# bruniss/multi-task-3d-resencoder-unet

Measured on AMD Instinct MI355X. Metric: train patches/sec (b,c,z,y,x) ResEncM 1x128^3, higher is better.
Workload: dtype bf16; 1 GPU; cfg2: ResEncM (6 stages, feats [32, 64, 128, 256, 512, 512], blocks [1, 3, 4, 6, 6, 6]), 1-in, heads ['sheet'], patch 128x128x128, batch 2/GPU, full train step (fwd+loss+bwd+allreduce+clip+AdamW); global_batch=2, parallelism=dp1

## Files before the change

### include/rxunet.h

```cpp
#ifndef RXUNET_H
#define RXUNET_H

#include <stddef.h>
#include <stdint.h>

#ifdef __cplusplus
extern "C" {
#endif

#define RX_OK 0
#define RX_EINVAL (-1)
#define RX_EUNSUPPORTED (-2)
#define RX_ELAUNCH (-3)
#define RX_EWORKSPACE (-4)

typedef enum { RX_F32 = 0, RX_BF16 = 1, RX_F16 = 2 } rx_dtype;
typedef enum { RX_ACT_NONE = 0, RX_ACT_SIGMOID = 1, RX_ACT_SOFTMAX = 2 } rx_head_act;

typedef struct {
  void* ptr;
  int32_t n, z, y, x, c, ld;
  int64_t cs;
} rx_act;

// ... 10 lines not shown
                  const int* taps, void* const* w_fwd, void* const* w_bwd, void* stream);

size_t rx_conv_workspace_hint(void);
int rx_conv3d_fwd(rx_dtype dt, const rx_act* x, const void* w_fwd, const float* bias, const rx_act* y,
                  const int32_t kernel[3], const int32_t stride[3], void* ws, size_t ws_bytes, void* stream);
int rx_conv3d_fwd_stats(rx_dtype dt, const rx_act* x, const void* w_fwd, const float* bias, const rx_act* y,
                        const int32_t kernel[3], const int32_t stride[3], float eps, float* stats, void* ws,
                        size_t ws_bytes, void* stream);
int rx_conv3d_bwd_data(rx_dtype dt, const rx_act* dy, const void* w_bwd, const rx_act* dx,
                       const int32_t kernel[3], const int32_t stride[3], int accumulate, void* ws,
                       size_t ws_bytes, void* stream);
int rx_conv3d_bwd_data_instats(rx_dtype dt, const rx_act* dy, const void* w_bwd, const rx_act* dx,
                               const int32_t kernel[3], const int32_t stride[3], int accumulate, const rx_act* in_y,
                               const float* in_stats, float slope, float* m12, int* fused, void* ws, size_t ws_bytes,
                               void* stream);
size_t rx_conv3d_bwd_weight_workspace(const rx_act* x, const rx_act* dy, const int32_t kernel[3]);
int rx_conv3d_bwd_weight(rx_dtype dt, const rx_act* x, const rx_act* dy, float* dw, const int32_t kernel[3],
                         const int32_t stride[3], void* ws, size_t ws_bytes, void* stream);

int rx_convT3d_fwd(rx_dtype dt, const rx_act* x, const void* w_fwd, const float* bias, const rx_act* y,
                   const int32_t stride[3], void* ws, size_t ws_bytes, void* stream);
int rx_convT3d_bwd_data(rx_dtype dt, const rx_act* dy, const void* w_bwd, const rx_act* dx,
                        const int32_t stride[3], int accumulate, void* ws, size_t ws_bytes, void* stream);
size_t rx_convT3d_bwd_weight_workspace(const rx_act* x, const rx_act* dy, const int32_t stride[3]);
int rx_convT3d_bwd_weight(rx_dtype dt, const rx_act* x, const rx_act* dy, float* dw, const int32_t stride[3],
                          void* ws, size_t ws_bytes, void* stream);

size_t rx_instnorm_stats_workspace(const rx_act* y);
int rx_instnorm_stats(rx_dtype dt, const rx_act* y, float eps, float* stats, void* ws, size_t ws_bytes,
                      void* stream);
// ... 249 lines not shown
```

### multi-task-3d-resencoder-unet_amd/csrc/build.py

```python
import os
import subprocess
import sys

HERE = os.path.dirname(os.path.abspath(__file__))
SOURCES = ["rx_runtime.hip", "rx_instnorm.hip", "rx_head.hip", "rx_stem.hip", "rx_pack_optim.hip", "rx_igemm.hip", "rx_wgrad.hip", "rx_wgrad_halo.hip", "rx_conv_halo.hip", "rx_stem_wgrad.hip", "rx_loss.hip", "rx_se.hip", "rx_dgrad_s2.hip", "rx_prog.hip", "rx_pointwise.hip", "rx_infer.hip", "rx_augment.hip", "rx_geometry.hip", "rx_morph.hip", "rx_patchsearch.hip", "rx_ingest.hip", "rx_affine.hip", "rx_metrics.hip", "rx_elastic.hip", "rx_preview.hip", "rx_meshslice.hip", "rx_surface.hip"]
HEADERS = ["rx_common.h", "rx_internal.h", "rx_reduce.h", "rx_instnorm_core.h", "rx_prog.h", "rx_affine_core.h", "rx_elastic_core.h", "rx_meshslice_core.h", "rx_conv_halo_plan.h", os.path.join("..", "..", "include", "rxunet.h")]
LIB = os.path.join(HERE, "librxunet.so")
HIPCC = os.environ.get("HIPCC", "/opt/rocm/bin/hipcc")
FLAGS = ["-O3", "--offload-arch=gfx950", "-std=c++17", "-fPIC", "-Wno-unused-result"]


def _stale(target, deps):
    if not os.path.exists(target):
        return True
    t = os.path.getmtime(target)
    return any(os.path.getmtime(d) > t for d in deps)


def build(force=False, verbose=True):
    hdrs = [os.path.join(HERE, h) for h in HEADERS] + [os.path.abspath(__file__)]
    objs = []
    procs = []
    for src in SOURCES:
        obj = os.path.join(HERE, src.replace(".hip", ".o"))
# ... 20 lines not shown
```

### multi-task-3d-resencoder-unet_amd/engine/lib.py

```python
import ctypes
import os
from ctypes import POINTER, c_char_p, c_double, c_float, c_int, c_int32, c_long, c_size_t, c_void_p

import torch

_HERE = os.path.dirname(os.path.abspath(__file__))
LIB_PATH = os.environ.get("RX_LIBRARY") or os.path.join(os.path.dirname(_HERE), "csrc", "librxunet.so")

RX_F32, RX_BF16, RX_F16 = 0, 1, 2
RX_ACT_NONE, RX_ACT_SIGMOID, RX_ACT_SOFTMAX = 0, 1, 2
DTYPE_CODE = {torch.float32: RX_F32, torch.bfloat16: RX_BF16, torch.float16: RX_F16}
RX_SW_U8, RX_SW_U16, RX_SW_F32 = 0, 1, 2
RX_SW_SCALE, RX_SW_ZSCORE = 0, 1
RX_SW_BLEND_AVERAGE, RX_SW_BLEND_UNIT, RX_SW_BLEND_NONE = 0, 1, 2
RX_SW_CAST_U8, RX_SW_CAST_U16 = 0, 1
RX_AUG_PW_NONE, RX_AUG_PW_AFFINE, RX_AUG_PW_PLANE, RX_AUG_PW_NOISE = 0, 1, 2, 3
RX_AUG_G3_NONE, RX_AUG_G3_FILTER, RX_AUG_G3_DOWNSCALE = 0, 1, 2
RX_AUG_MAX_K, RX_AUG_MAX_BOXES = 21, 4
RX_LOSS_BCE_LOGITS, RX_LOSS_BCE_PROB, RX_LOSS_MSE = 0, 1, 2
RX_REDUCE_MEAN, RX_REDUCE_SUM = 0, 1
RX_INGEST_COPY, RX_INGEST_DIV255, RX_INGEST_DIV65535, RX_INGEST_NORMAL_U16, RX_INGEST_NORMAL_MUL2 = 0, 1, 2, 3, 4
RX_AFFINE_LINEAR, RX_AFFINE_NEAREST = 0, 1
RX_AFFINE_CONSTANT, RX_AFFINE_CLAMP = 0, 1
RX_EDT_NONE, RX_EDT_MAX_EXTENT = 1 << 30, 1024
# ... 23 lines not shown

_SIGNATURES = {
    "rx_abi_version": (c_int, []),
    "rx_last_error": (c_char_p, []),
    "rx_device_arch_ok": (c_int, []),
    "rx_last_conv_kernel": (c_char_p, []),
    "rx_pack_conv_weight": (c_int, [c_int, c_void_p, c_int, c_int, c_int, c_void_p, c_void_p, c_void_p]),
    "rx_pack_convT_weight": (c_int, [c_int, c_void_p, c_int, c_int, c_int, c_void_p, c_void_p, c_void_p]),
    "rx_pack_multi": (c_int, [c_int, c_int, c_void_p, c_void_p, c_void_p, c_void_p, c_void_p, c_void_p, c_void_p, c_void_p]),
    "rx_conv_workspace_hint": (c_size_t, []),
    "rx_conv3d_fwd": (c_int, [c_int, _P, c_void_p, c_void_p, _P, I3, I3, c_void_p, c_size_t, c_void_p]),
    "rx_conv3d_fwd_stats": (c_int, [c_int, _P, c_void_p, c_void_p, _P, I3, I3, c_float, c_void_p, c_void_p, c_size_t, c_void_p]),
    "rx_conv3d_bwd_data": (c_int, [c_int, _P, c_void_p, _P, I3, I3, c_int, c_void_p, c_size_t, c_void_p]),
    "rx_conv3d_bwd_data_instats": (c_int, [c_int, _P, c_void_p, _P, I3, I3, c_int, _P, c_void_p, c_float, c_void_p, POINTER(c_int),
                                           c_void_p, c_size_t, c_void_p]),
    "rx_instnorm_act_bwd_apply": (c_int, [c_int, _P, _P, c_void_p, _P, c_float, c_void_p, _P, _P, c_int, c_void_p]),
    "rx_conv3d_bwd_weight_workspace": (c_size_t, [_P, _P, I3]),
    "rx_conv3d_bwd_weight": (c_int, [c_int, _P, _P, c_void_p, I3, I3, c_void_p, c_size_t, c_void_p]),
    "rx_convT3d_fwd": (c_int, [c_int, _P, c_void_p, c_void_p, _P, I3, c_void_p, c_size_t, c_void_p]),
    "rx_convT3d_bwd_data": (c_int, [c_int, _P, c_void_p, _P, I3, c_int, c_void_p, c_size_t, c_void_p]),
    "rx_convT3d_bwd_weight_workspace": (c_size_t, [_P, _P, I3]),
    "rx_convT3d_bwd_weight": (c_int, [c_int, _P, _P, c_void_p, I3, c_void_p, c_size_t, c_void_p]),
    "rx_instnorm_stats_workspace": (c_size_t, [_P]),
    "rx_instnorm_stats": (c_int, [c_int, _P, c_float, c_void_p, c_void_p, c_size_t, c_void_p]),
    "rx_instnorm_act_fwd": (c_int, [c_int, _P, c_void_p, _P, _P, c_float, c_void_p]),
    "rx_instnorm_stats_mask": (c_int, [c_void_p, c_void_p, c_int, c_void_p]),
    "rx_instnorm_fwd": (c_int, [c_int, _P, c_float, c_void_p, _P, _P, c_float, c_void_p, c_size_t, c_void_p]),
    "rx_instnorm_act_bwd": (c_int, [c_int, _P, _P, c_void_p, _P, c_float, _P, _P, c_int, c_void_p, c_size_t,
                                    c_void_p]),
    "rx_instnorm_act_bwd_res": (c_int, [c_int, _P, _P, c_void_p, _P, c_float, _P, I3, _P, _P, c_void_p, c_size_t, c_void_p]),
# ... 158 lines not shown
```

### multi-task-3d-resencoder-unet_amd/engine/ops/__init__.py

```python
from ctypes import byref, c_int32, c_void_p

import numpy as np
import torch

from .. import lib as _l
from ..lib import I3, RxAct, check, load, stream_ptr
from . import core, infer, losses, mesh, network, pipeline, validation
from .core import (_U16, Act, LaunchProfiler, Program, event_free, event_new, event_record, profiling,
                   set_profiler, stream_wait, timed_bytes, workspace)
from .infer import (SW_ACT, SW_BLEND, SW_CAST, SW_NORM, sw_accumulate, sw_finalize, sw_gather,
                    sw_gather_workspace, sw_occupancy)
from .losses import (bce_dice_loss_bwd, bce_dice_loss_fwd, cross_entropy_loss_bwd, cross_entropy_loss_fwd,
                     elem_loss_bwd, elem_loss_fwd, masked_cosine_loss_bwd, masked_cosine_loss_fwd)
from .mesh import mesh_slice_labels, mesh_slice_normals
from .network import (avgpool_bwd, avgpool_fwd, channel_sum, conv3d_bwd_data, conv3d_bwd_data_instats,
                      conv3d_bwd_weight, conv3d_fwd, conv3d_fwd_stats, convT3d_bwd_data, convT3d_bwd_weight, convT3d_fwd,
                      head_bwd, head_fwd, instnorm_act_bwd, instnorm_act_bwd_apply, instnorm_act_bwd_head,
                      instnorm_act_bwd_res, instnorm_act_fwd, instnorm_act_head_fwd, instnorm_act_pool_fwd, instnorm_fwd,
                      instnorm_gate_act_bwd, instnorm_gate_act_fwd, instnorm_stats, instnorm_stats_mask, pack_conv_weight,
                      pack_convT_weight, pack_weights_multi, se_gate_bwd, se_gate_fwd, se_workspace_bytes,
                      stem_conv_bwd_weight, stem_conv_fwd, stem_conv_fwd_stats)
from .pipeline import (affine_apply, affine_table, aug_filter_zy, aug_philox_u32, aug_pointwise, augment_batch,
                       box_stats, elastic_apply, elastic_nodes, elastic_tables, geom_apply, geom_table, ingest, label_dilate)
from .validation import (class_counts, edt_sq, mask_edges, normal_stats, preview_frames, preview_panel, seg_counts,
                         surface_hist, surface_scratch)
```

### multi-task-3d-resencoder-unet_amd/engine/ops/network.py

```python
import ctypes
from ctypes import byref, c_int

import torch

from .. import lib as _l
from ..lib import I3, check, load, stream_ptr
from .core import LaunchProfiler, _code, _desc, _ptr, _tb, _ws_args, flops, hbm, timed_bytes, workspace


def _pack_bytes(w, dtype, want_fwd, want_bwd):
    e = torch.empty((), dtype=dtype).element_size()
    return w.numel() * (4 + (e if want_fwd else 0) + (e if want_bwd else 0))


def _pack(entry, w, co, ci, dtype, w_fwd, w_bwd, want_fwd, want_bwd):
    taps = w[0, 0].numel()
    if want_fwd and w_fwd is None:
        w_fwd = torch.empty((taps, co, ci), dtype=dtype, device=w.device)
    if want_bwd and w_bwd is None:
        w_bwd = torch.empty((taps, ci, co), dtype=dtype, device=w.device)
    check(getattr(load(), entry)(_code(dtype), _ptr(w), w.shape[0], w.shape[1], taps, _ptr(w_fwd if want_fwd else None),
                                 _ptr(w_bwd if want_bwd else None), stream_ptr()), entry)
    return w_fwd, w_bwd

# ... 49 lines not shown
@flops(lambda dy, dx, kernel: _igemm("dgrad", dx, dy, dx, kernel))
def conv3d_bwd_data(dy, w_bwd, dx, kernel, stride, accumulate=False, ws=None):
    check(load().rx_conv3d_bwd_data(_code(dy.dtype), byref(dy.desc()), _ptr(w_bwd), byref(dx.desc()), I3(*kernel), I3(*stride),
                                    int(accumulate), *_ws_args(ws), stream_ptr()), "rx_conv3d_bwd_data")


@flops(lambda dy, dx, kernel: _igemm("dgrad", dx, dx, dy, kernel))
def conv3d_bwd_data_instats(dy, w_bwd, dx, kernel, stride, accumulate, in_y, in_stats, slope, m12, ws=None):
    fused = c_int(0)
    check(load().rx_conv3d_bwd_data_instats(_code(dy.dtype), byref(dy.desc()), _ptr(w_bwd), byref(dx.desc()), I3(*kernel),
                                            I3(*stride), int(accumulate), byref(in_y.desc()), _ptr(in_stats), float(slope),
                                            _ptr(m12), byref(fused), *_ws_args(ws), stream_ptr()), "rx_conv3d_bwd_data_instats")
    return bool(fused.value)


def _bwd_bytes(g, y, out, dy, d_residual, accumulate_residual):
    return _tb(g) + _tb(y) + _tb(dy) + _tb(out) + _tb(d_residual) * (2 if accumulate_residual else 1)


@hbm("in_act_bwd_apply", _bwd_bytes)
def instnorm_act_bwd_apply(g, y, stats, out, dy, m12, slope=0.01, d_residual=None, accumulate_residual=False):
    check(load().rx_instnorm_act_bwd_apply(_code(y.dtype), byref(g.desc()), byref(y.desc()), _ptr(stats), _desc(out), float(slope),
                                           _ptr(m12), byref(dy.desc()), _desc(d_residual), int(accumulate_residual), stream_ptr()),
          "rx_instnorm_act_bwd_apply")


@flops(lambda x, dy, kernel: (f"wgrad:wgrad_kernel<{64 if dy.c % 64 == 0 else 32},{64 if x.c % 64 == 0 else 32}>",
                              _conv_flops(dy, x, kernel)))
def conv3d_bwd_weight(x, dy, dw, kernel, stride, ws=None):
    need = load().rx_conv3d_bwd_weight_workspace(byref(x.desc()), byref(dy.desc()), I3(*kernel))
# ... 177 lines not shown
```

### multi-task-3d-resencoder-unet_amd/engine/plan.py

```python
import contextlib
import os
from dataclasses import dataclass
from typing import Callable, ClassVar, Dict, List, NamedTuple, Optional

import torch
from torch import nn

from . import lib as _l
from . import ops
from .ops import Act


class UnsupportedConfig(NotImplementedError):
    pass


_SIDE_STREAMS: Dict[str, "torch.cuda.Stream"] = {}


def side_stream(device):
    key = str(device)
    st = _SIDE_STREAMS.get(key)
    if st is None:
        st = _SIDE_STREAMS[key] = torch.cuda.Stream(device=device)
# ... 82 lines not shown


@dataclass(eq=False)
class ConvRec:
    kind: ClassVar[str] = "conv"
    x: AT
    y: AT
    pk: dict
    b: Optional[torch.Tensor]
    widx: int
    bidx: Optional[int]
    kernel: list
    stride: list
    stats_to: Optional["InactRec"] = None
    instats_for: Optional["InactRec"] = None


@dataclass(eq=False)
class ConvTRec:
    kind: ClassVar[str] = "convT"
    x: AT
    y: AT
    pk: dict
    b: Optional[torch.Tensor]
    widx: int
    bidx: Optional[int]
    stride: list
    cat: AT


@dataclass(eq=False)
class InactRec:
    kind: ClassVar[str] = "inact"
    y: AT
    stats: torch.Tensor
    eps: float
    res: Optional[AT]
    out: AT
    slope: float
    gate: Optional[Gate]
    drop: Optional[Drop]
    stats_done: bool = False
    pool_to: Optional["PoolRec"] = None
    head_to: Optional["HeadRec"] = None
    head_src: Optional["HeadRec"] = None
    head_dw_fused: bool = False
    m12: Optional[torch.Tensor] = None
    m12_valid: bool = False
    m12x: Optional[torch.Tensor] = None


@dataclass(eq=False)
class PoolRec:
    kind: ClassVar[str] = "pool"
    x: AT
    y: AT
    stride: list
# ... 489 lines not shown
                                [((slice(None), slice(0, head.in_channels)), (slice(None), slice(None)))])
            tape.append(HeadRec(x=low, w=hw_k, b=head.bias, widx=self._param(head.weight), bidx=self._param(head.bias), k=k,
                                name=name, out=out, act=act_code))

        self._gen_forward()
        if self.needs_grad:
            self._gen_backward()

    def _fuse_conv_stats(self, tape):
        for rec, nxt in zip(tape, tape[1:]):
            if (rec.kind == "conv" and nxt.kind == "inact" and nxt.y is rec.y and self.dtype != torch.float32
                    and list(rec.kernel) == [3, 3, 3] and list(rec.stride) == [1, 1, 1]
                    and _above_single_launch(rec.y.act) and _halo_x_ok(rec.y.act)):
                rec.stats_to, nxt.stats_done = nxt, True

    def _fuse_stem_stats(self, tape):
        for rec, nxt in zip(tape, tape[1:]):
            if (rec.kind == "stem" and nxt.kind == "inact" and nxt.y is rec.y and self.dtype != torch.float32
                    and _above_single_launch(rec.y.act)):
                rec.stats_to, nxt.stats_done = nxt, True

    def _fuse_block_pool(self, tape):
        producers = {id(r.out): r for r in tape if r.kind == "inact" and r.gate is None}
        for rec in tape:
            if rec.kind == "pool" and id(rec.x) in producers and _above_single_launch(rec.x.act):
                src = producers[id(rec.x)]
                if src.pool_to is None:
                    src.pool_to, rec.fused = rec, True

    def _fuse_head(self, tape):
# ... 15 lines not shown
        def step():
            st = r.stats_to
            if st is not None:
                ops.stem_conv_fwd_stats(self._x, r.w, r.b, r.y.act, r.kernel, st.stats, self._eps_now(st))
                self._mask_dropped(st)
            else:
                ops.stem_conv_fwd(self._x, r.w, r.b, r.y.act, r.kernel)
        return [step]

    def _fwd_image(self, r: ImageRec):
        return [lambda: ops.stem_conv_fwd(self._x, r.w, None, r.y.act, [1, 1, 1])]

    def _fwd_conv(self, r: ConvRec):
        def step():
            self._await_pack(r.pk)
            st = r.stats_to
            if st is not None:
                ops.conv3d_fwd_stats(r.x.act, r.pk["w_fwd"], r.b, r.y.act, r.kernel, r.stride, st.stats, self._eps_now(st))
                self._mask_dropped(st)
            else:
                ops.conv3d_fwd(r.x.act, r.pk["w_fwd"], r.b, r.y.act, r.kernel, r.stride)
        return [step]

    def _fwd_convT(self, r: ConvTRec):
        def step():
            self._await_pack(r.pk)
            ops.convT3d_fwd(r.x.act, r.pk["w_fwd"], r.b, r.y.act, r.stride)
        return [step]

    def _fwd_inact(self, r: InactRec):
        res = r.res.act if r.res is not None else None
        g, head, pool = r.gate, r.head_to, r.pool_to
# ... 18 lines not shown
            ops.instnorm_act_head_fwd(r.y.act, r.stats, r.out.act if keep else None, head.w.view(head.k, -1), head.b, head.out,
                                      head.act if self._apply_act else _l.RX_ACT_NONE, r.slope)

        def with_pool():
            stats_pass()
            ops.instnorm_act_pool_fwd(r.y.act, r.stats, r.out.act, pool.y.act, pool.stride, r.slope, res)

        def plain():
            if r.stats_done:
                ops.instnorm_act_fwd(r.y.act, r.stats, r.out.act, r.slope, res)
            elif r.drop is not None and r.drop.active:
                stats_pass()
                ops.instnorm_act_fwd(r.y.act, r.stats, r.out.act, r.slope, res)
            else:
                ops.instnorm_fwd(r.y.act, r.stats, r.out.act, r.slope, res, r.eps)
        if g is not None:
            return [gated]
        return [with_head if head is not None else with_pool if pool is not None else plain]

    def _fwd_pool(self, r: PoolRec):
        return [] if r.fused else [lambda: ops.avgpool_fwd(r.x.act, r.y.act, r.stride)]

    def _fwd_copy(self, r: CopyRec):
        return [lambda: ops.avgpool_fwd(r.x.act, r.y.act, (1, 1, 1))]

    def _fwd_head(self, r: HeadRec):
        if r.fwd_fused:
            return []
        return [lambda: ops.head_fwd(r.x.act, r.w.view(r.k, -1), r.b, r.out, r.act if self._apply_act else _l.RX_ACT_NONE)]

# ... 1 lines not shown
        f = self.fwd
        self.n_fwd_enc = None
        self.fwd_dec_start = []
        build = {StemRec: self._fwd_stem, ImageRec: self._fwd_image, ConvRec: self._fwd_conv, ConvTRec: self._fwd_convT,
                 InactRec: self._fwd_inact, PoolRec: self._fwd_pool, CopyRec: self._fwd_copy, HeadRec: self._fwd_head}
        full_res = self.spatial[0] * self.spatial[1] * self.spatial[2]
        for tape in [self.enc_tape] + self.dec_tapes:
            if tape is not self.enc_tape:
                if self.n_fwd_enc is None:
                    self.n_fwd_enc = len(f)
                self.fwd_dec_start.append(len(f))
            self._fuse_conv_stats(tape)
            self._fuse_stem_stats(tape)
            self._fuse_block_pool(tape)
            self._fuse_head(tape)
            for rec in tape:
                if (tape is self.enc_tape and self._pack_delay_at is None and rec.kind in ("conv", "pool")
                        and rec.y.act.voxels < full_res):
                    self._pack_delay_at = len(f)
                f += build[type(rec)](rec)

    def _dy_for(self, y: AT):
        key = (y.act.dims, y.act.c)
        turn = self._dy_turn.get(key, 0)
        self._dy_turn[key] = (turn + 1) % self.dy_ring
        slot = key + (turn,)
        if slot not in self.dy_pool:
            t = torch.empty((*y.act.dims, y.act.c), dtype=self.dtype, device=self.device)
            self.bytes_alloc += t.numel() * t.element_size()
            self.dy_pool[slot] = Act(t)
# ... 105 lines not shown
        gres, acc = None, False
        if res is not None and res.needs_grad:
            gres, acc = self._claim_grad(res, r)
        plain16 = r.gate is None and res is None and self.dtype != torch.float32 and _above_single_launch(out.act)
        last = out.last_writer
        if plain16 and isinstance(last, HeadRec):
            heads = [h for h in tape if h.kind == "head" and h.x is out]
            if len(heads) == 1 and heads[0].k <= 4:
                r.head_src, last.dx_fused = heads[0], True
                if heads[0].fwd_fused and heads[0].w is self.params[heads[0].widx]:
                    r.head_dw_fused, last.dw_fused = True, True
        if (plain16 and isinstance(last, ConvRec) and out.act.full_buffer and out.act.root is None and out.act.c % 32 == 0
                and _halo_x_ok(out.act)):
            r.m12 = torch.empty((self.B, out.act.c, 2), dtype=torch.float32, device=self.device)
            last.instats_for = r
        if r.gate is not None:
            return [self._bwd_inact_gated(r, gout, dy, gres, acc)]
        pend, out.pool_pending = out.pool_pending, None
        if gres is not None and not acc and _above_single_launch(y.act):
            return [self._bwd_inact_res(r, gout, dy, gres, pend)]
        steps = []
        if pend is not None:
            steps.append(lambda: ops.avgpool_bwd(pend.gy, pend.gx, pend.stride, True))
        return steps + [self._bwd_inact_plain(r, gout, dy, gres, acc)]

    def _bwd_inact_gated(self, r, gout, dy, gres, acc):
        g = r.gate

        def step():
            self._before_dy_write(dy)
# ... 51 lines not shown
        def wlaunch(dw, ws):
            if r.kind == "stem":
                ops.stem_conv_bwd_weight(self._x, dy, dw, r.kernel, ws)
            elif "wgrad" not in self._skip:
                ops.conv3d_bwd_weight(r.x.act, dy, dw, r.kernel, r.stride, ws)
        steps = [self._wgrad_step(r, dy, wlaunch)]
        if r.kind == "conv" and r.x.needs_grad:
            gx, acc = self._claim_grad(r.x, r)
            if r.x.act.full_buffer:
                self._cat_written[r.x.act.key] = True

            def dstep():
                if "dgrad" in self._skip:
                    return
                ia = r.instats_for
                if ia is None:
                    ops.conv3d_bwd_data(dy, r.pk["w_bwd"], gx, r.kernel, r.stride, acc)
                else:
                    ia.m12_valid = ops.conv3d_bwd_data_instats(dy, r.pk["w_bwd"], gx, r.kernel, r.stride, acc, ia.y.act, ia.stats,
                                                               ia.slope, ia.m12)
            steps.append(dstep)
        return steps

    def _bwd_convT(self, r: ConvTRec, tape, i):
        if not self._view_written(r.y):
            raise RuntimeError("plan bug: concat gradient not initialised before the transposed conv")
        gy = self._cat_grad(r)
        gx, acc = self._claim_grad(r.x, r)
        wstep = self._wgrad_step(r, gy, lambda dw, ws: ops.convT3d_bwd_weight(r.x.act, gy, dw, r.stride, ws))

        def step():
# ... 465 lines not shown
```

Before: 117.0 patches/s.

## Add fused small-volume conv+instnorm kernels for deep low-resolution stages

Adds a dedicated HIP kernel for 3x3x3 stride-1 convs on volumes of at most 64 voxels. One workgroup holds a whole sample's activations in LDS, splits K across waves, and fuses the instance-norm statistics plus normalize/activation/residual into the forward conv. In backward, the dgrad kernel is fused with the preceding instnorm backward and residual-gradient accumulation. The aim is to remove separate launches and round trips through memory at the tiny 4^3 bottleneck stages. The cost is a new code path whose grid parallelism is small (N*Co/16 blocks), so it could underuse the GPU.

```diff
diff --git a/include/rxunet.h b/include/rxunet.h
--- a/include/rxunet.h
+++ b/include/rxunet.h
@@ -48,6 +48,15 @@
                                const int32_t kernel[3], const int32_t stride[3], int accumulate, const rx_act* in_y,
                                const float* in_stats, float slope, float* m12, int* fused, void* ws, size_t ws_bytes,
                                void* stream);
+int rx_conv_small_select(rx_dtype dt, int z, int y, int x, int ci, int co, const int32_t kernel[3],
+                         const int32_t stride[3]);
+int rx_conv3d_in_fwd_small(rx_dtype dt, const rx_act* x, const void* w_fwd, const float* bias, const rx_act* y,
+                           const int32_t kernel[3], const int32_t stride[3], float eps, float* stats,
+                           const rx_act* residual, const rx_act* out, float slope, void* stream);
+int rx_conv3d_bwd_data_in_small(rx_dtype dt, const rx_act* dy, const void* w_bwd, const rx_act* dx,
+                                const int32_t kernel[3], const int32_t stride[3], int accumulate, const rx_act* in_y,
+                                const float* in_stats, const rx_act* in_out, float slope, const rx_act* in_dy,
+                                const rx_act* d_residual, int accumulate_residual, void* stream);
 size_t rx_conv3d_bwd_weight_workspace(const rx_act* x, const rx_act* dy, const int32_t kernel[3]);
 int rx_conv3d_bwd_weight(rx_dtype dt, const rx_act* x, const rx_act* dy, float* dw, const int32_t kernel[3],
                          const int32_t stride[3], void* ws, size_t ws_bytes, void* stream);
diff --git a/multi-task-3d-resencoder-unet_amd/csrc/build.py b/multi-task-3d-resencoder-unet_amd/csrc/build.py
--- a/multi-task-3d-resencoder-unet_amd/csrc/build.py
+++ b/multi-task-3d-resencoder-unet_amd/csrc/build.py
@@ -3,7 +3,7 @@
 import sys
 
 HERE = os.path.dirname(os.path.abspath(__file__))
-SOURCES = ["rx_runtime.hip", "rx_instnorm.hip", "rx_head.hip", "rx_stem.hip", "rx_pack_optim.hip", "rx_igemm.hip", "rx_wgrad.hip", "rx_wgrad_halo.hip", "rx_conv_halo.hip", "rx_stem_wgrad.hip", "rx_loss.hip", "rx_se.hip", "rx_dgrad_s2.hip", "rx_prog.hip", "rx_pointwise.hip", "rx_infer.hip", "rx_augment.hip", "rx_geometry.hip", "rx_morph.hip", "rx_patchsearch.hip", "rx_ingest.hip", "rx_affine.hip", "rx_metrics.hip", "rx_elastic.hip", "rx_preview.hip", "rx_meshslice.hip", "rx_surface.hip"]
+SOURCES = ["rx_runtime.hip", "rx_instnorm.hip", "rx_head.hip", "rx_stem.hip", "rx_pack_optim.hip", "rx_igemm.hip", "rx_conv_small.hip", "rx_wgrad.hip", "rx_wgrad_halo.hip", "rx_conv_halo.hip", "rx_stem_wgrad.hip", "rx_loss.hip", "rx_se.hip", "rx_dgrad_s2.hip", "rx_prog.hip", "rx_pointwise.hip", "rx_infer.hip", "rx_augment.hip", "rx_geometry.hip", "rx_morph.hip", "rx_patchsearch.hip", "rx_ingest.hip", "rx_affine.hip", "rx_metrics.hip", "rx_elastic.hip", "rx_preview.hip", "rx_meshslice.hip", "rx_surface.hip"]
 HEADERS = ["rx_common.h", "rx_internal.h", "rx_reduce.h", "rx_instnorm_core.h", "rx_prog.h", "rx_affine_core.h", "rx_elastic_core.h", "rx_meshslice_core.h", "rx_conv_halo_plan.h", os.path.join("..", "..", "include", "rxunet.h")]
 LIB = os.path.join(HERE, "librxunet.so")
 HIPCC = os.environ.get("HIPCC", "/opt/rocm/bin/hipcc")
diff --git a/multi-task-3d-resencoder-unet_amd/csrc/rx_conv_small.hip b/multi-task-3d-resencoder-unet_amd/csrc/rx_conv_small.hip
--- /dev/null
+++ b/multi-task-3d-resencoder-unet_amd/csrc/rx_conv_small.hip
@@ -0,0 +1,409 @@
+#include "rx_common.h"
+#include "rx_internal.h"
+#include "rx_reduce.h"
+#include "rx_instnorm_core.h"
+
+constexpr int CS_MAXV = 64;
+constexpr int CS_BN = 16;
+constexpr int CS_NW = 8;
+constexpr int CS_RING = 8;
+constexpr int CS_KU = 64;
+constexpr int CS_MAXCI = 1024;
+constexpr int CS_STAGE = 16 * CS_KU * 2;
+
+struct CsArgs {
+  const void* in;
+  const void* w;
+  int ldi;
+  long in_ss;
+  int Z, Y, X, V, Ci, Co, N, flip;
+  void* o;
+  int ldo;
+  long o_ss;
+  const float* bias;
+  int accumulate;
+  float* stats_w;
+  const float* stats_r;
+  float eps, slope;
+  const void* res;
+  int ldr;
+  long r_ss;
+  void* out;
+  int ldout;
+  long out_ss;
+  const void* iy;
+  int ldiy;
+  long iy_ss;
+  const void* iout;
+  int ldio;
+  long io_ss;
+  void* dy;
+  int lddy;
+  long dy_ss;
+  void* dres;
+  int lddr;
+  long dr_ss;
+  int acc_res, mask;
+};
+
+template <typename T>
+struct Mma16;
+template <>
+struct Mma16<bf16_t> {
+  __device__ static inline void run(f32x4& c, const u32x4& a, const u32x4& b) {
+    c = __builtin_amdgcn_mfma_f32_16x16x32_bf16(__builtin_bit_cast(bf16x8, a), __builtin_bit_cast(bf16x8, b), c, 0, 0, 0);
+  }
+};
+template <>
+struct Mma16<f16_t> {
+  __device__ static inline void run(f32x4& c, const u32x4& a, const u32x4& b) {
+    c = __builtin_amdgcn_mfma_f32_16x16x32_f16(__builtin_bit_cast(f16x8, a), __builtin_bit_cast(f16x8, b), c, 0, 0, 0);
+  }
+};
+
+template <typename T>
+struct alignas(8) Vec8 {
+  T v[4];
+};
+template <typename T>
+__device__ inline Vec8<T> ld8(const T* p) {
+  Vec8<T> r;
+  *reinterpret_cast<u32x2*>(&r) = *reinterpret_cast<const u32x2*>(p);
+  return r;
+}
+template <typename T>
+__device__ inline void st8(T* p, const Vec8<T>& r) {
+  *reinterpret_cast<u32x2*>(p) = *reinterpret_cast<const u32x2*>(&r);
+}
+
+static size_t cs_lds_main(int Ci) {
+  const size_t act = (size_t)(CS_MAXV + 1) * Ci * 2 + (size_t)CS_NW * CS_STAGE, part = (size_t)CS_NW * CS_MAXV * CS_BN * sizeof(float);
+  return act > part ? act : part;
+}
+static size_t cs_lds_bytes(int Ci) { return cs_lds_main(Ci) + 4 * 2 * CS_BN * sizeof(double) + 2 * CS_BN * sizeof(float); }
+
+template <typename T, bool BWD>
+__global__ __launch_bounds__(CS_NW * 64) void conv_small_kernel(const CsArgs a, int lds_main) {
+  extern __shared__ __attribute__((aligned(16))) unsigned char cs_smem[];
+  u32x4* sX = reinterpret_cast<u32x4*>(cs_smem);
+  float* part = reinterpret_cast<float*>(cs_smem);
+  double* red = reinterpret_cast<double*>(cs_smem + lds_main);
+  float* pr = reinterpret_cast<float*>(cs_smem + lds_main + 4 * 2 * CS_BN * sizeof(double));
+
+  const int tid = threadIdx.x, lane = tid & 63, wave = __builtin_amdgcn_readfirstlane(tid >> 6);
+  const int lid = rx_xcd_remap(blockIdx.x, gridDim.x);
+  const int n = lid % a.N, co0 = (lid / a.N) * CS_BN;
+  const int X8 = a.Ci >> 3, nkc = a.Ci / CS_KU, rowb = a.Ci * 2;
+  const int swm = (X8 & 15) ? 7 : 15;
+  const int U = 27 * nkc;
+  const int ubeg = U * wave / CS_NW, cnt = U * (wave + 1) / CS_NW - ubeg;
+  const T* in_n = reinterpret_cast<const T*>(a.in) + (long)n * a.in_ss;
+  const T* wl = reinterpret_cast<const T*>(a.w) + (long)(co0 + (lane >> 3)) * a.Ci + (lane & 7) * 8;
+  const long wtap = (long)a.Co * a.Ci;
+
+  u32x4 wr[CS_RING][2];
+  int ltap = ubeg / nkc, lcc = ubeg % nkc;
+  auto load_unit = [&](u32x4 (&dst)[2]) {
+    const int tap = ltap < 27 ? ltap : 26;
+    const T* p = wl + tap * wtap + lcc * CS_KU;
+    dst[0] = *reinterpret_cast<const u32x4*>(p);
+    dst[1] = *reinterpret_cast<const u32x4*>(p + 8 * a.Ci);
+    if (++lcc == nkc) lcc = 0, ++ltap;
+  };
+#pragma unroll
+  for (int i = 0; i < CS_RING; ++i) load_unit(wr[i]);
+
+  {
+    const int nchunk = a.V * X8;
+    for (int base = 0; base < nchunk; base += CS_NW * 64 * 8) {
+      u32x4 t[8];
+#pragma unroll
+      for (int i = 0; i < 8; ++i) {
+        int idx = base + i * CS_NW * 64 + tid;
+        idx = idx < nchunk ? idx : nchunk - 1;
+        const int u = idx / X8, c = idx - u * X8;
+        t[i] = *reinterpret_cast<const u32x4*>(in_n + (long)u * a.ldi + c * 8);
+      }
+#pragma unroll
+      for (int i = 0; i < 8; ++i) {
+        const int idx = base + i * CS_NW * 64 + tid;
+        const int u = idx / X8, c = idx - u * X8;
+        if (idx < nchunk) sX[u * X8 + (c ^ (u & swm))] = t[i];
+      }
+    }
+    if (tid < X8) sX[CS_MAXV * X8 + tid] = u32x4{0u, 0u, 0u, 0u};
+  }
+
+  const int sgn = a.flip ? -1 : 1;
+  const int zrow = CS_MAXV * rowb;
+  int vox[4];
+  unsigned pm[4];
+#pragma unroll
+  for (int b = 0; b < 4; ++b) {
+    const int v = b * 16 + (lane & 15);
+    vox[b] = v;
+    const int vx = v % a.X, t = v / a.X;
+    const int vy = t % a.Y, vz = t / a.Y;
+    unsigned m = 0;
+#pragma unroll
+    for (int d = 0; d < 3; ++d) {
+      const int o = sgn * (d - 1);
+      m |= ((unsigned)(vz + o) < (unsigned)a.Z ? 1u : 0u) << d;
+      m |= ((unsigned)(vy + o) < (unsigned)a.Y ? 8u : 0u) << d;
+      m |= ((unsigned)(vx + o) < (unsigned)a.X ? 64u : 0u) << d;
+    }
+    pm[b] = v < a.V ? m : 0u;
+  }
+  int ra[4], sw16[4];
+  auto set_tap = [&](int tap) {
+    const int tz = tap / 9, ty = (tap / 3) % 3, tx = tap % 3;
+    const unsigned need = (1u << tz) | (8u << ty) | (64u << tx);
+    const int delta = sgn * (((tz - 1) * a.Y + (ty - 1)) * a.X + (tx - 1));
+#pragma unroll
+    for (int b = 0; b < 4; ++b) {
+      const bool ok = (pm[b] & need) == need;
+      const int src = vox[b] + delta;
+      ra[b] = ok ? src * rowb : zrow;
+      sw16[b] = ok ? (src & swm) << 4 : 0;
+    }
+  };
+  f32x4 acc[4];
+#pragma unroll
+  for (int b = 0; b < 4; ++b) acc[b] = f32x4{0.f, 0.f, 0.f, 0.f};
+  __syncthreads();
+
+  const int h = lane >> 4;
+  unsigned char* stage = cs_smem + (CS_MAXV + 1) * rowb + wave * CS_STAGE;
+  const int wrow = lane >> 3;
+  unsigned char* st0 = stage + wrow * 128 + (((lane & 7) ^ ((wrow >> 1) & 7)) << 4);
+  unsigned char* st1 = stage + (wrow + 8) * 128 + (((lane & 7) ^ (((wrow >> 1) & 7) ^ 4)) << 4);
+  const int frow = lane & 15;
+  const unsigned char* fr0 = stage + frow * 128 + ((h ^ ((frow >> 1) & 7)) << 4);
+  const unsigned char* fr1 = stage + frow * 128 + (((h + 4) ^ ((frow >> 1) & 7)) << 4);
+  int ctap = ubeg / nkc, ccc = ubeg % nkc;
+  set_tap(ctap);
+  u32x4 aq[2][2], bq[2][8];
+  auto fetch = [&](u32x4 (&slot)[2], u32x4 (&af)[2], u32x4 (&bf)[8], bool live) {
+    *reinterpret_cast<u32x4*>(st0) = slot[0];
+    *reinterpret_cast<u32x4*>(st1) = slot[1];
+    af[0] = *reinterpret_cast<const u32x4*>(fr0);
+    af[1] = *reinterpret_cast<const u32x4*>(fr1);
+    const int c16 = ccc * 128 + h * 16;
+#pragma unroll
+    for (int b = 0; b < 4; ++b) {
+      const int ad = (live ? ra[b] : zrow) + (c16 ^ sw16[b]);
+      bf[2 * b] = *reinterpret_cast<const u32x4*>(cs_smem + ad);
+      bf[2 * b + 1] = *reinterpret_cast<const u32x4*>(cs_smem + (ad ^ 64));
+    }
+    if (++ccc == nkc) {
+      ccc = 0, ++ctap;
+      set_tap(ctap < 27 ? ctap : 26);
+    }
+    load_unit(slot);
+  };
+  fetch(wr[0], aq[0], bq[0], true);
+  for (int kb = 0; kb < cnt; kb += CS_RING) {
+#pragma unroll
+    for (int i = 0; i < CS_RING; ++i) {
+      fetch(wr[(i + 1) % CS_RING], aq[(i + 1) & 1], bq[(i + 1) & 1], kb + i + 1 < cnt);
+#pragma unroll
+      for (int b = 0; b < 4; ++b) Mma16<T>::run(acc[b], aq[i & 1][0], bq[i & 1][2 * b]);
+#pragma unroll
+      for (int b = 0; b < 4; ++b) Mma16<T>::run(acc[b], aq[i & 1][1], bq[i & 1][2 * b + 1]);
+    }
+  }
+
+  __syncthreads();
+#pragma unroll
+  for (int b = 0; b < 4; ++b) *reinterpret_cast<f32x4*>(part + ((wave * 64 + b * 16 + (lane & 15)) * CS_BN + 4 * h)) = acc[b];
+  __syncthreads();
+
+  const int v = tid >> 2, cq = tid & 3, c = co0 + 4 * cq;
+  const bool act = tid < 256 && v < a.V;
+  float s[4] = {0.f, 0.f, 0.f, 0.f}, q[4] = {0.f, 0.f, 0.f, 0.f};
+  Vec8<T> ov;
+  float gg[4], xh[4], mean[4], rstd[4];
+  T* op = reinterpret_cast<T*>(a.o) + (long)n * a.o_ss + (long)v * a.ldo + c;
+  if (act) {
+    f32x4 f = *reinterpret_cast<const f32x4*>(part + (v * CS_BN + 4 * cq));
+#pragma unroll
+    for (int w = 1; w < CS_NW; ++w) f += *reinterpret_cast<const f32x4*>(part + ((w * 64 + v) * CS_BN + 4 * cq));
+    if (!BWD) {
+      if (a.bias) f += *reinterpret_cast<const f32x4*>(a.bias + c);
+    } else if (a.accumulate) {
+      const Vec8<T> old = ld8(op);
+#pragma unroll
+      for (int j = 0; j < 4; ++j) f[j] += Elem<T>::to_f(old.v[j]);
+    }
+#pragma unroll
+    for (int j = 0; j < 4; ++j) ov.v[j] = Elem<T>::from_f(f[j]);
+    st8(op, ov);
+    if (!BWD) {
+#pragma unroll
+      for (int j = 0; j < 4; ++j) {
+        const float t = Elem<T>::to_f(ov.v[j]);
+        s[j] += t;
+        q[j] += t * t;
+      }
+    } else {
+      load_pair(a.stats_r, n, a.Co, c, mean, rstd);
+      const Vec8<T> yv = ld8(reinterpret_cast<const T*>(a.iy) + (long)n * a.iy_ss + (long)v * a.ldiy + c);
+      Vec8<T> mv;
+      if (a.mask == IN_MASK_OUT) mv = ld8(reinterpret_cast<const T*>(a.iout) + (long)n * a.io_ss + (long)v * a.ldio + c);
+#pragma unroll
+      for (int j = 0; j < 4; ++j) {
+        xh[j] = in_xhat(yv.v[j], mean[j], rstd[j]);
+        gg[j] = Elem<T>::to_f(ov.v[j]);
+        in_bwd_gprime(gg[j], xh[j], (InMask)a.mask, mv.v[j], a.slope);
+        s[j] += gg[j];
+        q[j] += gg[j] * xh[j];
+      }
+    }
+  }
+  if (tid < 256) {
+    for (int o = 4; o < 64; o <<= 1) {
+#pragma unroll
+      for (int j = 0; j < 4; ++j) {
+        s[j] += __shfl_xor(s[j], o, 64);
+        q[j] += __shfl_xor(q[j], o, 64);
+      }
+    }
+    if (lane < 4) {
+#pragma unroll
+      for (int j = 0; j < 4; ++j) {
+        red[(wave * 2 + 0) * CS_BN + lane * 4 + j] = (double)s[j];
+        red[(wave * 2 + 1) * CS_BN + lane * 4 + j] = (double)q[j];
+      }
+    }
+  }
+  __syncthreads();
+  if (tid < CS_BN) {
+    const double s0 = red[0 * CS_BN + tid] + red[2 * CS_BN + tid] + red[4 * CS_BN + tid] + red[6 * CS_BN + tid];
+    const double s1 = red[1 * CS_BN + tid] + red[3 * CS_BN + tid] + red[5 * CS_BN + tid] + red[7 * CS_BN + tid];
+    if (!BWD) {
+      double mu = s0 / a.V, var = s1 / a.V - mu * mu;
+      if (var < 0.0) var = 0.0;
+      const float m = (float)mu, r = (float)(1.0 / sqrt(var + (double)a.eps));
+      pr[tid] = m;
+      pr[CS_BN + tid] = r;
+      a.stats_w[2 * ((size_t)n * a.Co + co0 + tid)] = m;
+      a.stats_w[2 * ((size_t)n * a.Co + co0 + tid) + 1] = r;
+    } else {
+      pr[tid] = (float)(s0 / a.V);
+      pr[CS_BN + tid] = (float)(s1 / a.V);
+    }
+  }
+  __syncthreads();
+  if (!act) return;
+  if (!BWD) {
+    Vec8<T> rv, o;
+    if (a.res) rv = ld8(reinterpret_cast<const T*>(a.res) + (long)n * a.r_ss + (long)v * a.ldr + c);
+#pragma unroll
+    for (int j = 0; j < 4; ++j) {
+      const float m = pr[4 * cq + j], r = pr[CS_BN + 4 * cq + j];
+      o.v[j] = a.res ? in_fwd_elem<T, true>(ov.v[j], m, r, rv.v[j], a.slope) : in_fwd_elem<T, false>(ov.v[j], m, r, rv.v[j], a.slope);
+    }
+    st8(reinterpret_cast<T*>(a.out) + (long)n * a.out_ss + (long)v * a.ldout + c, o);
+  } else {
+    Vec8<T> dv, rv;
+    T* rp = reinterpret_cast<T*>(a.dres) + (long)n * a.dr_ss + (long)v * a.lddr + c;
+    if (a.dres && a.acc_res) rv = ld8(rp);
+#pragma unroll
+    for (int j = 0; j < 4; ++j) {
+      dv.v[j] = Elem<T>::from_f(in_bwd_dy(gg[j], xh[j], rstd[j], pr[4 * cq + j], pr[CS_BN + 4 * cq + j]));
+      if (a.dres) {
+        float r = gg[j];
+        if (a.acc_res) r += Elem<T>::to_f(rv.v[j]);
+        rv.v[j] = Elem<T>::from_f(r);
+      }
+    }
+    st8(reinterpret_cast<T*>(a.dy) + (long)n * a.dy_ss + (long)v * a.lddy + c, dv);
+    if (a.dres) st8(rp, rv);
+  }
+}
+
+
+extern "C" int rx_conv_small_select(rx_dtype dt, int z, int y, int x, int ci, int co, const int32_t kernel[3], const int32_t stride[3]) {
+  if (!kernel || !stride) RX_FAIL(RX_EINVAL, "rx_conv_small_select: bad arguments");
+  if (dt != RX_BF16 && dt != RX_F16) RX_FAIL(RX_EUNSUPPORTED, "conv_small: 16-bit compute types only (fp32 keeps the split-K summation order)");
+  for (int i = 0; i < 3; ++i)
+    if (kernel[i] != 3 || stride[i] != 1) RX_FAIL(RX_EUNSUPPORTED, "conv_small: 3x3x3 stride-1 layers only");
+  if (z < 1 || y < 1 || x < 1 || (long)z * y * x > CS_MAXV)
+    RX_FAIL(RX_EUNSUPPORTED, "conv_small: at most %d voxels per sample (got %d x %d x %d)", CS_MAXV, z, y, x);
+  if (ci < CS_KU || ci % CS_KU || ci > CS_MAXCI) RX_FAIL(RX_EUNSUPPORTED, "conv_small: input channels must be a multiple of %d, at most %d (got %d)", CS_KU, CS_MAXCI, ci);
+  if (co < 32 || co % 32) RX_FAIL(RX_EUNSUPPORTED, "conv_small: output channels must be a multiple of 32 (got %d)", co);
+  return RX_OK;
+}
+
+template <bool BWD>
+static int cs_launch(rx_dtype dt, const CsArgs& a, hipStream_t st) {
+  const size_t lds = cs_lds_bytes(a.Ci);
+  const int lds_main = (int)cs_lds_main(a.Ci);
+  const dim3 grid(a.N * (a.Co / CS_BN)), block(CS_NW * 64);
+  rx_note_kernel(BWD ? "conv_small_dgrad_in" : "conv_small_fwd_in");
+  if (dt == RX_BF16) {
+    (void)hipFuncSetAttribute(reinterpret_cast<const void*>(&conv_small_kernel<bf16_t, BWD>), hipFuncAttributeMaxDynamicSharedMemorySize, (int)lds);
+    hipLaunchKernelGGL((conv_small_kernel<bf16_t, BWD>), grid, block, lds, st, a, lds_main);
+  } else {
+    (void)hipFuncSetAttribute(reinterpret_cast<const void*>(&conv_small_kernel<f16_t, BWD>), hipFuncAttributeMaxDynamicSharedMemorySize, (int)lds);
+    hipLaunchKernelGGL((conv_small_kernel<f16_t, BWD>), grid, block, lds, st, a, lds_main);
+  }
+  return RX_OK;
+}
+
+static void cs_geom(CsArgs& a, const rx_act* in, const void* w, const rx_act* o, int flip) {
+  memset(&a, 0, sizeof(a));
+  a.in = in->ptr, a.w = w, a.ldi = in->ld, a.in_ss = rx_act_voxels(in) * (long)in->ld;
+  a.Z = o->z, a.Y = o->y, a.X = o->x, a.V = (int)rx_act_voxels(o), a.Ci = in->c, a.Co = o->c, a.N = o->n, a.flip = flip;
+  a.o = o->ptr, a.ldo = o->ld, a.o_ss = rx_act_voxels(o) * (long)o->ld;
+}
+
+extern "C" int rx_conv3d_in_fwd_small(rx_dtype dt, const rx_act* x, const void* w_fwd, const float* bias, const rx_act* y,
+                                      const int32_t kernel[3], const int32_t stride[3], float eps, float* stats, const rx_act* residual,
+                                      const rx_act* out, float slope, void* stream) {
+  RX_RECORD(stream, [=, x_ = RxActV(x), y_ = RxActV(y), kernel_ = RxI3V(kernel), stride_ = RxI3V(stride), residual_ = RxActV(residual), out_ = RxActV(out)](void* s) { return rx_conv3d_in_fwd_small(dt, x_.p(), w_fwd, bias, y_.p(), kernel_.v, stride_.v, eps, stats, residual_.p(), out_.p(), slope, s); });
+  if (!w_fwd || !stats || !kernel || !stride) RX_FAIL(RX_EINVAL, "rx_conv3d_in_fwd_small: bad arguments");
+  int rc = check_vec_channels(x, dt, "rx_conv3d_in_fwd_small(x)", CS_MAXCI);
+  if (rc) return rc;
+  if ((rc = check_acts(dt, "rx_conv3d_in_fwd_small", y, {{"y", y, true}, {"out", out, true}, {"residual", residual, false}}))) return rc;
+  if (x->n != y->n || x->z != y->z || x->y != y->y || x->x != y->x) RX_FAIL(RX_EINVAL, "rx_conv3d_in_fwd_small: output geometry mismatch");
+  if ((rc = rx_conv_small_select(dt, y->z, y->y, y->x, x->c, y->c, kernel, stride))) return rc;
+  if (((uintptr_t)w_fwd & 15) || (bias && ((uintptr_t)bias & 15))) RX_FAIL(RX_EUNSUPPORTED, "rx_conv3d_in_fwd_small: misaligned weights / bias");
+  CsArgs a;
+  cs_geom(a, x, w_fwd, y, 0);
+  a.bias = bias, a.stats_w = stats, a.eps = eps, a.slope = slope;
+  if (residual) a.res = residual->ptr, a.ldr = residual->ld, a.r_ss = rx_act_voxels(residual) * (long)residual->ld;
+  a.out = out->ptr, a.ldout = out->ld, a.out_ss = rx_act_voxels(out) * (long)out->ld;
+  cs_launch<false>(dt, a, (hipStream_t)stream);
+  RX_CHECK_LAUNCH("rx_conv3d_in_fwd_small");
+  return RX_OK;
+}
+
+extern "C" int rx_conv3d_bwd_data_in_small(rx_dtype dt, const rx_act* dy, const void* w_bwd, const rx_act* dx, const int32_t kernel[3],
+                                           const int32_t stride[3], int accumulate, const rx_act* in_y, const float* in_stats,
+                                           const rx_act* in_out, float slope, const rx_act* in_dy, const rx_act* d_residual,
+                                           int accumulate_residual, void* stream) {
+  RX_RECORD(stream, [=, dy_ = RxActV(dy), dx_ = RxActV(dx), kernel_ = RxI3V(kernel), stride_ = RxI3V(stride), in_y_ = RxActV(in_y), in_out_ = RxActV(in_out), in_dy_ = RxActV(in_dy), d_residual_ = RxActV(d_residual)](void* s) { return rx_conv3d_bwd_data_in_small(dt, dy_.p(), w_bwd, dx_.p(), kernel_.v, stride_.v, accumulate, in_y_.p(), in_stats, in_out_.p(), slope, in_dy_.p(), d_residual_.p(), accumulate_residual, s); });
+  if (!w_bwd || !in_stats || !kernel || !stride) RX_FAIL(RX_EINVAL, "rx_conv3d_bwd_data_in_small: bad arguments");
+  const InMask mask = in_mask_of(slope, in_out);
+  int rc = check_vec_channels(dy, dt, "rx_conv3d_bwd_data_in_small(dy)", CS_MAXCI);
+  if (rc) return rc;
+  if ((rc = check_acts(dt, "rx_conv3d_bwd_data_in_small", dx, {{"dx", dx, true}, {"in_y", in_y, true}, {"in_dy", in_dy, true},
+                       {"in_out", mask == IN_MASK_OUT ? in_out : nullptr, false}, {"d_residual", d_residual, false}})))
+    return rc;
+  if (dy->n != dx->n || dy->z != dx->z || dy->y != dx->y || dy->x != dx->x) RX_FAIL(RX_EINVAL, "rx_conv3d_bwd_data_in_small: geometry mismatch");
+  if ((rc = rx_conv_small_select(dt, dx->z, dx->y, dx->x, dy->c, dx->c, kernel, stride))) return rc;
+  if ((uintptr_t)w_bwd & 15) RX_FAIL(RX_EUNSUPPORTED, "rx_conv3d_bwd_data_in_small: misaligned weights");
+  if (in_dy->ptr == dx->ptr || (d_residual && (d_residual->ptr == dx->ptr || d_residual->ptr == in_dy->ptr)))
+    RX_FAIL(RX_EINVAL, "rx_conv3d_bwd_data_in_small: dx, in_dy and d_residual must be different buffers");
+  CsArgs a;
+  cs_geom(a, dy, w_bwd, dx, 1);
+  a.accumulate = accumulate, a.stats_r = in_stats, a.slope = slope, a.mask = (int)mask;
+  a.iy = in_y->ptr, a.ldiy = in_y->ld, a.iy_ss = rx_act_voxels(in_y) * (long)in_y->ld;
+  if (mask == IN_MASK_OUT) a.iout = in_out->ptr, a.ldio = in_out->ld, a.io_ss = rx_act_voxels(in_out) * (long)in_out->ld;
+  a.dy = in_dy->ptr, a.lddy = in_dy->ld, a.dy_ss = rx_act_voxels(in_dy) * (long)in_dy->ld;
+  if (d_residual) a.dres = d_residual->ptr, a.lddr = d_residual->ld, a.dr_ss = rx_act_voxels(d_residual) * (long)d_residual->ld, a.acc_res = accumulate_residual;
+  cs_launch<true>(dt, a, (hipStream_t)stream);
+  RX_CHECK_LAUNCH("rx_conv3d_bwd_data_in_small");
+  return RX_OK;
+}
diff --git a/multi-task-3d-resencoder-unet_amd/engine/lib.py b/multi-task-3d-resencoder-unet_amd/engine/lib.py
--- a/multi-task-3d-resencoder-unet_amd/engine/lib.py
+++ b/multi-task-3d-resencoder-unet_amd/engine/lib.py
@@ -61,6 +61,10 @@
     "rx_conv3d_bwd_data": (c_int, [c_int, _P, c_void_p, _P, I3, I3, c_int, c_void_p, c_size_t, c_void_p]),
     "rx_conv3d_bwd_data_instats": (c_int, [c_int, _P, c_void_p, _P, I3, I3, c_int, _P, c_void_p, c_float, c_void_p, POINTER(c_int),
                                            c_void_p, c_size_t, c_void_p]),
+    "rx_conv_small_select": (c_int, [c_int, c_int, c_int, c_int, c_int, c_int, I3, I3]),
+    "rx_conv3d_in_fwd_small": (c_int, [c_int, _P, c_void_p, c_void_p, _P, I3, I3, c_float, c_void_p, _P, _P, c_float, c_void_p]),
+    "rx_conv3d_bwd_data_in_small": (c_int, [c_int, _P, c_void_p, _P, I3, I3, c_int, _P, c_void_p, _P, c_float, _P, _P, c_int,
+                                            c_void_p]),
     "rx_instnorm_act_bwd_apply": (c_int, [c_int, _P, _P, c_void_p, _P, c_float, c_void_p, _P, _P, c_int, c_void_p]),
     "rx_conv3d_bwd_weight_workspace": (c_size_t, [_P, _P, I3]),
     "rx_conv3d_bwd_weight": (c_int, [c_int, _P, _P, c_void_p, I3, I3, c_void_p, c_size_t, c_void_p]),
diff --git a/multi-task-3d-resencoder-unet_amd/engine/ops/__init__.py b/multi-task-3d-resencoder-unet_amd/engine/ops/__init__.py
--- a/multi-task-3d-resencoder-unet_amd/engine/ops/__init__.py
+++ b/multi-task-3d-resencoder-unet_amd/engine/ops/__init__.py
@@ -13,7 +13,8 @@
 from .losses import (bce_dice_loss_bwd, bce_dice_loss_fwd, cross_entropy_loss_bwd, cross_entropy_loss_fwd,
                      elem_loss_bwd, elem_loss_fwd, masked_cosine_loss_bwd, masked_cosine_loss_fwd)
 from .mesh import mesh_slice_labels, mesh_slice_normals
-from .network import (avgpool_bwd, avgpool_fwd, channel_sum, conv3d_bwd_data, conv3d_bwd_data_instats,
+from .network import (avgpool_bwd, avgpool_fwd, channel_sum, conv3d_bwd_data, conv3d_bwd_data_in_small,
+                      conv3d_bwd_data_instats, conv3d_in_fwd_small, conv_small_ok,
                       conv3d_bwd_weight, conv3d_fwd, conv3d_fwd_stats, convT3d_bwd_data, convT3d_bwd_weight, convT3d_fwd,
                       head_bwd, head_fwd, instnorm_act_bwd, instnorm_act_bwd_apply, instnorm_act_bwd_head,
                       instnorm_act_bwd_res, instnorm_act_fwd, instnorm_act_head_fwd, instnorm_act_pool_fwd, instnorm_fwd,
diff --git a/multi-task-3d-resencoder-unet_amd/engine/ops/network.py b/multi-task-3d-resencoder-unet_amd/engine/ops/network.py
--- a/multi-task-3d-resencoder-unet_amd/engine/ops/network.py
+++ b/multi-task-3d-resencoder-unet_amd/engine/ops/network.py
@@ -87,6 +87,26 @@
     return bool(fused.value)
 
 
+def conv_small_ok(x, y, kernel, stride):
+    return x.dims == y.dims and load().rx_conv_small_select(_code(y.dtype), *y.dims[1:], x.c, y.c, I3(*kernel), I3(*stride)) == 0
+
+
+@flops(lambda x, y, kernel: ("fwd:conv_small_fwd_in", _conv_flops(y, x, kernel)))
+def conv3d_in_fwd_small(x, w_fwd, bias, y, kernel, stride, stats, out, slope=0.01, residual=None, eps=1e-5):
+    check(load().rx_conv3d_in_fwd_small(_code(x.dtype), byref(x.desc()), _ptr(w_fwd), _ptr(bias), byref(y.desc()), I3(*kernel),
+                                        I3(*stride), float(eps), _ptr(stats), _desc(residual), byref(out.desc()), float(slope),
+                                        stream_ptr()), "rx_conv3d_in_fwd_small")
+
+
+@flops(lambda dy, dx, kernel: ("dgrad:conv_small_dgrad_in", _conv_flops(dx, dy, kernel)))
+def conv3d_bwd_data_in_small(dy, w_bwd, dx, kernel, stride, accumulate, in_y, in_stats, in_out, in_dy, slope=0.01, d_residual=None,
+                             accumulate_residual=False):
+    check(load().rx_conv3d_bwd_data_in_small(_code(dy.dtype), byref(dy.desc()), _ptr(w_bwd), byref(dx.desc()), I3(*kernel), I3(*stride),
+                                             int(accumulate), byref(in_y.desc()), _ptr(in_stats), _desc(in_out), float(slope),
+                                             byref(in_dy.desc()), _desc(d_residual), int(accumulate_residual), stream_ptr()),
+          "rx_conv3d_bwd_data_in_small")
+
+
 def _bwd_bytes(g, y, out, dy, d_residual, accumulate_residual):
     return _tb(g) + _tb(y) + _tb(dy) + _tb(out) + _tb(d_residual) * (2 if accumulate_residual else 1)
 
diff --git a/multi-task-3d-resencoder-unet_amd/engine/plan.py b/multi-task-3d-resencoder-unet_amd/engine/plan.py
--- a/multi-task-3d-resencoder-unet_amd/engine/plan.py
+++ b/multi-task-3d-resencoder-unet_amd/engine/plan.py
@@ -120,6 +120,8 @@
     stride: list
     stats_to: Optional["InactRec"] = None
     instats_for: Optional["InactRec"] = None
+    inact_to: Optional["InactRec"] = None
+    inbwd_below: Optional[Callable] = None
 
 
 @dataclass(eq=False)
@@ -147,6 +149,7 @@
     gate: Optional[Gate]
     drop: Optional[Drop]
     stats_done: bool = False
+    by_conv: bool = False
     pool_to: Optional["PoolRec"] = None
     head_to: Optional["HeadRec"] = None
     head_src: Optional["HeadRec"] = None
@@ -666,6 +669,13 @@
                     and _above_single_launch(rec.y.act) and _halo_x_ok(rec.y.act)):
                 rec.stats_to, nxt.stats_done = nxt, True
 
+    def _fuse_conv_inact_small(self, tape):
+        for rec, nxt in zip(tape, tape[1:]):
+            if (rec.kind == "conv" and nxt.kind == "inact" and nxt.y is rec.y and nxt.gate is None and nxt.drop is None
+                    and nxt.pool_to is None and nxt.head_to is None and not rec.x.act.is_planar_cat
+                    and ops.conv_small_ok(rec.x.act, rec.y.act, rec.kernel, rec.stride)):
+                rec.inact_to, nxt.by_conv = nxt, True
+
     def _fuse_stem_stats(self, tape):
         for rec, nxt in zip(tape, tape[1:]):
             if (rec.kind == "stem" and nxt.kind == "inact" and nxt.y is rec.y and self.dtype != torch.float32
@@ -711,8 +721,11 @@
     def _fwd_conv(self, r: ConvRec):
         def step():
             self._await_pack(r.pk)
-            st = r.stats_to
-            if st is not None:
+            st, ia = r.stats_to, r.inact_to
+            if ia is not None:
+                ops.conv3d_in_fwd_small(r.x.act, r.pk["w_fwd"], r.b, r.y.act, r.kernel, r.stride, ia.stats, ia.out.act, ia.slope,
+                                        ia.res.act if ia.res is not None else None, ia.eps)
+            elif st is not None:
                 ops.conv3d_fwd_stats(r.x.act, r.pk["w_fwd"], r.b, r.y.act, r.kernel, r.stride, st.stats, self._eps_now(st))
                 self._mask_dropped(st)
             else:
@@ -761,6 +774,8 @@
                 ops.instnorm_act_fwd(r.y.act, r.stats, r.out.act, r.slope, res)
             else:
                 ops.instnorm_fwd(r.y.act, r.stats, r.out.act, r.slope, res, r.eps)
+        if r.by_conv:
+            return []
         if g is not None:
             return [gated]
         return [with_head if head is not None else with_pool if pool is not None else plain]
@@ -792,6 +807,7 @@
             self._fuse_stem_stats(tape)
             self._fuse_block_pool(tape)
             self._fuse_head(tape)
+            self._fuse_conv_inact_small(tape)
             for rec in tape:
                 if (tape is self.enc_tape and self._pack_delay_at is None and rec.kind in ("conv", "pool")
                         and rec.y.act.voxels < full_res):
@@ -927,6 +943,16 @@
                 and _halo_x_ok(out.act)):
             r.m12 = torch.empty((self.B, out.act.c, 2), dtype=torch.float32, device=self.device)
             last.instats_for = r
+        if (r.gate is None and r.head_src is None and out.pool_pending is None and isinstance(last, ConvRec) and last.x is out
+                and out.act.full_buffer and out.act.root is None and ops.conv_small_ok(last.y.act, out.act, last.kernel, last.stride)):
+            mask_out = out.act if (r.slope != 1.0 and res is not None) else None
+
+            def below(dy_up, w_bwd, acc_up):
+                self._before_dy_write(dy)
+                ops.conv3d_bwd_data_in_small(dy_up, w_bwd, gout, last.kernel, last.stride, acc_up, y.act, r.stats, mask_out, dy,
+                                             r.slope, gres, acc)
+            last.inbwd_below = below
+            return []
         if r.gate is not None:
             return [self._bwd_inact_gated(r, gout, dy, gres, acc)]
         pend, out.pool_pending = out.pool_pending, None
@@ -1008,7 +1034,9 @@
                 if "dgrad" in self._skip:
                     return
                 ia = r.instats_for
-                if ia is None:
+                if r.inbwd_below is not None:
+                    r.inbwd_below(dy, r.pk["w_bwd"], acc)
+                elif ia is None:
                     ops.conv3d_bwd_data(dy, r.pk["w_bwd"], gx, r.kernel, r.stride, acc)
                 else:
                     ia.m12_valid = ops.conv3d_bwd_data_instats(dy, r.pk["w_bwd"], gx, r.kernel, r.stride, acc, ia.y.act, ia.stats,
```

New measurement: 117.7 patches/s, median of 6. Within noise of the previous version (+0.5%).
